# ha7ilm/csdr

Measured on AMD Instinct MI355X. Metric: complex MS/s in->out, WFM demod chain @2.4 MS/s x N streams, higher is better.
Workload: dtype f32

## Files before the change

### csdr_amd/csrc/wfm.hip

```cpp
#include "common.hpp"
#include "wfm_mfma.hpp"
#include "seeds.hpp"
#include <math.h>
#include <stdlib.h>
#include <vector>
#include <string>
#include <string.h>
using namespace csdr_amd;

namespace {

constexpr int HIST = WFM_HIST;
constexpr int TILE_A = 64;
constexpr int WARM = 48;

struct WfmParams {
    int D, L, F;
    int T;
    long long B;
    long long j_first;
    int n_audio;
};

__device__ __forceinline__ float u8_to_f(uint32_t v) { return fmaf((float)v, 0x1.010102p-7f, -1.0f); }
// ... 147 lines not shown
    long long B, next_j;
    int last_T, flip;
    bool ended;
    std::string kernel_name;
    bool profiling;
    std::vector<std::pair<hipEvent_t, hipEvent_t>> ev_pool;
    size_t ev_used;
    double prof_ms; long prof_launches;
    bool use_mfma;
    WfmMfmaDevice mfma;
    float2 *d_ctab; size_t ctab_cap;
    float2 c_prev;
    long long tab_first; bool tab_valid;
    bool ps; std::vector<float> rates, h_taps; csdr_amd::SeedTables *seeds; float *d_scales;
    float2 *d_dtab_old; int *d_list, *d_lead_n; float *d_lead_d; std::vector<int> retuned;
};

extern "C" {

static int wfm_upload_stream_tables(csdr_amd_wfm *w, int s, float rate)
{
    WfmMfmaTable t;
    wfm_mfma_build_table(w->D, w->L, w->F, rate, w->h_taps.data(), t);
    CSDR_HIP(hipMemcpy((uint8_t *)w->mfma.d_seq_frags + (size_t)s * t.seq_frags.size(), t.seq_frags.data(), t.seq_frags.size(), hipMemcpyHostToDevice));
    CSDR_HIP(hipMemcpy(w->mfma.d_seq_cum + (size_t)s * t.seq_cum.size(), t.seq_cum.data(), t.seq_cum.size() * sizeof(float), hipMemcpyHostToDevice));
    CSDR_HIP(hipMemcpy(w->mfma.d_dtab + (size_t)s * t.dtab.size(), t.dtab.data(), t.dtab.size() * sizeof(float2), hipMemcpyHostToDevice));
    CSDR_HIP(hipMemcpy(w->d_scales + s, &t.seq_scale, sizeof(float), hipMemcpyHostToDevice));
    return 0;
}

// ... 3 lines not shown
    const float shift_rate = rates ? rates[0] : 0.f;
    if (n_streams <= 0 || decimation <= 0 || taps_length <= 0 || frac_rate <= 1 || !rates) { fail_msg(-3, "wfm: bad parameters"); return nullptr; }
    if (decimation * 1 + taps_length + 8 > HIST) { fail_msg(-3, "wfm: D + taps (%d + %d) exceed the %d-sample history", decimation, taps_length, HIST); return nullptr; }
    if (max_block_samples < 1024) max_block_samples = 1024;
    csdr_amd_wfm *w = new csdr_amd_wfm();
    w->ctx = ctx; w->n_streams = n_streams; w->D = decimation; w->L = taps_length; w->F = frac_rate; w->audio_rate = audio_rate;
    w->shift_rate = shift_rate; w->tau = tau; w->max_block = max_block_samples;
    const float dt = (float)(1.0 / audio_rate); w->alpha = dt / (tau + dt);
    const size_t max_audio = max_block_samples / ((size_t)decimation * frac_rate) + 8;
    w->demod_pitch = (max_audio + 40 + 63) & ~(size_t)63;
    hipError_t e = hipSuccess;
    auto alloc = [&](void **p, size_t bytes) { if (e == hipSuccess) e = hipMalloc(p, bytes); };
    w->d_demod = nullptr; w->d_rot = nullptr; w->d_hist = nullptr; w->d_head[0] = w->d_head[1] = nullptr; w->hflip = 0;
    w->use_mfma = false; w->d_ctab = nullptr; w->ctab_cap = 0; w->mfma.d_seq_frags = nullptr; w->mfma.d_seq_cum = nullptr; w->mfma.d_dtab = nullptr;
    w->ps = per_stream; w->seeds = nullptr; w->d_scales = nullptr; w->d_dtab_old = nullptr; w->d_list = nullptr; w->d_lead_n = nullptr; w->d_lead_d = nullptr;
    {
        const char *force = getenv("CSDR_AMD_WFM_PATH");
        w->use_mfma = !(force && !strcmp(force, "valu")) && wfm_mfma_supported(decimation, taps_length, frac_rate);
    }
    if (per_stream && !w->use_mfma) { fail_msg(-3, "wfm_create_rates: a rate per stream needs the matrix-core chain kernel (decimation x audio decimation even, window <= 256 samples)"); delete w; return nullptr; }
    alloc((void **)&w->d_taps, sizeof(float) * taps_length);
    alloc((void **)&w->d_last[0], sizeof(float) * n_streams);
    alloc((void **)&w->d_last[1], sizeof(float) * n_streams);
    if (w->use_mfma) {
        alloc((void **)&w->d_head[0], wfm_mfma_head_bytes(n_streams));
        alloc((void **)&w->d_head[1], wfm_mfma_head_bytes(n_streams));
    } else {
        alloc((void **)&w->d_demod, sizeof(float) * w->demod_pitch * n_streams);
        alloc((void **)&w->d_rot, sizeof(cf32) * (HIST + max_block_samples + 64));
        alloc((void **)&w->d_hist, (size_t)2 * HIST * n_streams);
    }
    if (e != hipSuccess) { fail(e, "hipMalloc(wfm state)", __FILE__, __LINE__); csdr_amd_wfm_destroy(w); return nullptr; }
    (void)hipMemcpy(w->d_taps, host_taps, sizeof(float) * taps_length, hipMemcpyHostToDevice);
    w->kernel_name = "k_wfm_front";
    if (w->use_mfma && per_stream) {
        WfmMfmaTable t;
        wfm_mfma_build_table(decimation, taps_length, frac_rate, shift_rate, host_taps, t);
        w->mfma.tile_stride_bytes = t.tile_stride_bytes; w->mfma.win_off_bytes = t.win_off_bytes; w->mfma.seq_scale = t.seq_scale;
        w->rates.assign(rates, rates + n_streams); w->h_taps.assign(host_taps, host_taps + taps_length);
        hipError_t e2 = hipMalloc(&w->mfma.d_seq_frags, t.seq_frags.size() * (size_t)n_streams);
        if (e2 == hipSuccess) e2 = hipMalloc((void **)&w->mfma.d_seq_cum, t.seq_cum.size() * sizeof(float) * (size_t)n_streams);
// ... 51 lines not shown
    }
    const int rc = wfm_upload_stream_tables(w, stream, shift_rate); if (rc) return rc;
    w->rates[stream] = shift_rate;
    return seeds_set_rate(w->seeds, stream, shift_rate, false);
}

float csdr_amd_wfm_get_rate(const csdr_amd_wfm *w, int stream) { return w->ps ? ((stream >= 0 && stream < w->n_streams) ? w->rates[stream] : 0.f) : w->shift_rate; }

void csdr_amd_wfm_destroy(csdr_amd_wfm *w)
{
    if (!w) return;
    (void)hipStreamSynchronize(w->ctx->stream);
    if (w->seeds) seeds_destroy(w->seeds);
    (void)hipFree(w->d_scales); (void)hipFree(w->d_dtab_old); (void)hipFree(w->d_lead_n); (void)hipFree(w->d_lead_d);
    (void)hipFree(w->d_taps); (void)hipFree(w->d_demod); (void)hipFree(w->d_last[0]); (void)hipFree(w->d_last[1]);
    (void)hipFree(w->d_rot); (void)hipFree(w->d_hist); (void)hipFree(w->d_head[0]); (void)hipFree(w->d_head[1]);
    for (auto &pr : w->ev_pool) { (void)hipEventDestroy(pr.first); (void)hipEventDestroy(pr.second); }
    (void)hipFree(w->mfma.d_seq_frags); (void)hipFree(w->mfma.d_seq_cum); (void)hipFree(w->mfma.d_dtab); (void)hipFree(w->d_ctab);
    delete w;
}

int csdr_amd_wfm_reset(csdr_amd_wfm *w)
{
    hipStream_t st = w->ctx->stream;
    w->phase = 0.f;
    CSDR_HIP(hipMemsetAsync(w->d_last[0], 0, sizeof(float) * w->n_streams, st));
    CSDR_HIP(hipMemsetAsync(w->d_last[1], 0, sizeof(float) * w->n_streams, st));
    if (w->d_rot) CSDR_HIP(hipMemsetAsync(w->d_rot, 0, sizeof(cf32) * (HIST + w->max_block + 64), st));
    if (w->d_hist) CSDR_HIP(hipMemsetAsync(w->d_hist, 0x80, (size_t)2 * HIST * w->n_streams, st));
    for (int k = 0; k < 2; k++) if (w->d_head[k]) CSDR_HIP(hipMemsetAsync(w->d_head[k], 0x80, wfm_mfma_head_bytes(w->n_streams), st));
    w->hflip = 0;
// ... 113 lines not shown
                if (n_lead > n_audio) n_lead = n_audio;
            }
            if (n_lead > 0) {
                const int nr = (int)w->retuned.size(), S = w->n_streams;
                if (!w->d_lead_n) { CSDR_HIP(hipMalloc((void **)&w->d_lead_n, sizeof(int) * 2 * S)); w->d_list = w->d_lead_n + S; CSDR_HIP(hipMalloc((void **)&w->d_lead_d, sizeof(float) * (size_t)lead_max * S)); }
                int *hl = (int *)c->pinned_acquire(sizeof(int) * (size_t)(S + nr)); if (!hl) return -2;
                for (int s = 0; s < S; s++) hl[s] = 0;
                for (int k = 0; k < nr; k++) { hl[w->retuned[k]] = (int)n_lead; hl[S + k] = w->retuned[k]; }
                rc = c->pinned_upload(w->d_lead_n, sizeof(int) * (size_t)(S + nr)); if (rc) return rc;
                rc = wfm_mfma_lead(st, in, in_pitch, back.head_in, w->d_taps, sv.ctab, sv.pitch, w->mfma.d_dtab, w->d_dtab_old, w->d_list, nr, w->d_lead_d, lead_max,
                                   w->D, w->L, w->F, w->B, w->next_j, (int)n_lead);
                if (rc) return rc;
                psa.d_lead_d = w->d_lead_d; psa.d_lead_n = w->d_lead_n;
            }
        }
        rc = wfm_mfma_launch(st, e0, e1, in, in_pitch, w->mfma, ctab_call, w->n_streams, T, w->B, w->next_j, n_audio, back, w->ps ? &psa : nullptr);
        if (rc) return rc;
        if (n_audio > 0) w->retuned.clear();
        w->hflip ^= 1;
        if (n_audio > 0) w->flip ^= 1;
    } else {
        if ((size_t)n_audio + 40 > w->demod_pitch) return fail_msg(-3, "wfm: internal audio buffer too small");
        if (n_audio > 0) {
            WfmParams p; p.D = w->D; p.L = w->L; p.F = w->F; p.T = T; p.B = w->B; p.j_first = w->next_j; p.n_audio = n_audio;
            const int span = w->D * (w->F * (TILE_A - 1) + 1) + w->L + 16;
            const size_t lds = (size_t)((span + 7) / 8 * 8 + 2 * TILE_A) * sizeof(float2) + 64;
            if (lds > 64 * 1024) { const int arc = lds_attr_once((const void *)k_wfm_front, lds); if (arc) return arc; }
            if (e0) CSDR_HIP(hipEventRecord(e0, st));
            hipLaunchKernelGGL(k_wfm_front, dim3(w->n_streams, cdiv(n_audio, TILE_A)), dim3(256), lds, st,
                               in, in_pitch, w->d_hist, w->d_rot, w->d_taps, w->d_demod, w->demod_pitch, p);
            CSDR_LAUNCH_CHECK();
// ... 18 lines not shown
```

### csdr_amd/csrc/wfm_mfma.hip

```cpp
#include "common.hpp"
#include "wfm_mfma.hpp"
#include <hip/hip_ext.h>
#include <math.h>
#include <string.h>
#include <stdlib.h>
#include <complex>
#include <vector>
using namespace csdr_amd;

namespace csdr_amd {

bool wfm_mfma_supported(int D, int L, int F)
{
    if ((D * F) & 1) return false;
    const int win_off = (18 * D) & ~15;
    const int span_bytes = 2 * (D * (3 * F + 10) + L) - win_off;
    if (span_bytes > 64 * WFM_NK) return false;
    if (D + L + 3 * D * F + 8 > WFM_HIST) return false;
    return true;
}

void wfm_mfma_build_table(int D, int L, int F, float shift_rate, const float *taps, WfmMfmaTable &t)
{
    t.D = D; t.L = L; t.F = F;
// ... 97 lines not shown
            for (int l = 0; l < 3; l++) acc[l] = __builtin_amdgcn_mfma_i32_16x16x64_i8(A[ks * 3 + l], Bf[ks], acc[l], 0, 0, 0);
        }
    }
}

struct SeqParams {
    int n_streams; long long B2; long long tile_first; int n_tiles, tiles_per_seg;
    int stride, win_off; float scale;
    long long two_T;
    float alpha; const float *last_in; float *last_out; int16_t *s16; float *af; size_t out_pitch; long long j_first; int n_audio;
    const uint8_t *head_in; uint8_t *head_out;
    long long col_bytes; int col_chunks, col_audio, n_cols;
    size_t frag_stride, tab_pitch; int tab_len;
    const float *scales;
    const float *lead_d; const int *lead_n; int lead_stride;
};

#ifndef SEQ_RB_KIB
#define SEQ_RB_KIB 9
#endif
constexpr int SEQ_RB = 1024 * SEQ_RB_KIB;
#ifndef SEQ_RING_PAD
#define SEQ_RING_PAD 32
#endif
constexpr int SEQ_RP = SEQ_RB + SEQ_RING_PAD;
constexpr int SEQ_NGR = 4 * WFM_NK;
#ifndef SEQ_TPG_N
#define SEQ_TPG_N 6
#endif
#ifndef SEQ_NLD_N
// ... 4 lines not shown
constexpr int SEQ_NW = SEQ_TPG + SEQ_NLD;
constexpr int SEQ_NLW = SEQ_NLD;
constexpr int SEQ_LINE = 64;
constexpr int SEQ_OUTS = (SEQ_LINE - 1 + 3 * 4 * SEQ_TPG + 4 * SEQ_TPG - 1) / (4 * SEQ_TPG);
constexpr int SEQ_OUTR = SEQ_OUTS * 4 * SEQ_TPG;
constexpr int SEQ_OUTP = SEQ_OUTR + 4;
static_assert(16 % SEQ_NLW == 0 && (16 / SEQ_NLW) * 7 <= 63 && SEQ_TPG % 2 == 0, "rows per fetching wave (vmcnt counts to 63); the de-emphasis scan works on pairs");
constexpr int SEQ_HEAD = 1024;

#ifndef WFM_DIAG
#define WFM_DIAG 0
#endif
#ifdef WFM_PROF
__device__ unsigned long long g_wfm_prof[SEQ_NW][8];
__device__ unsigned long long g_wfm_life[SEQ_NW][4];
#define PROF_T(k) { const long long t_now = __builtin_readcyclecounter(); prof[k] += t_now - t_prev; t_prev = t_now; }
#else
#define PROF_T(k)
#endif

constexpr int RES_WARM = 48;
struct ResCtl {
    const uint32_t *desc;
    const uint32_t *ctrl;
    uint32_t *done;
    unsigned *cnt;
    unsigned long long *t_first;
    unsigned long long *next_item;
    unsigned *exiting;
    const uint8_t *in_ring; int16_t *out_ring; size_t in_slot_bytes, out_slot_elems;
    int n_slots, desc_lines, n_wsb, T, D, L, F;
    long long idle_ticks, life_ticks;
    const float *lead_d; int lead_stride;
    const float *lead_state;
    unsigned long long *stats;
    int fence_mode;
};
__device__ __forceinline__ uint32_t sys_load(const uint32_t *p) { return __hip_atomic_load(p, __ATOMIC_RELAXED, __HIP_MEMORY_SCOPE_SYSTEM); }
__device__ __forceinline__ uint32_t res_tag(long long k) { return (uint32_t)((unsigned long long)k % 0xfffffffeull) + 1u; }

template <bool PS, bool RES = false>
__global__ __launch_bounds__(64 * SEQ_NW) void k_wfm_mfma_seq(const uint8_t *__restrict__ in, size_t in_pitch, const v4i *__restrict__ frags, const float *__restrict__ cum,
                                                               const float2 *__restrict__ dtab, const float2 *__restrict__ ctab, SeqParams p_in, ResCtl rc)
{
    static_assert(!(PS && RES), "the resident form exists for the shared-rate kernel");
    constexpr int TPG = SEQ_TPG, SPW = 16 / SEQ_NLW, NTHR = 64 * SEQ_NW;
    extern __shared__ float4 lds_raw[];
    uint8_t *lds_in = reinterpret_cast<uint8_t *>(lds_raw);
    float *lds_out = reinterpret_cast<float *>(lds_in + 16 * SEQ_RP);
    float *lcum = lds_out + 16 * SEQ_OUTP;
    float2 *ctl = reinterpret_cast<float2 *>(lcum + (SEQ_NGR + 1) * 16);
    const int tid = threadIdx.x, wv = __builtin_amdgcn_readfirstlane(tid >> 6), lane = tid & 63, col = lane & 15, q = lane >> 4;
    const bool fetches = wv >= TPG;
#ifdef WFM_PROF
    const long long t_entry = __builtin_readcyclecounter();
    long long t_first = t_entry, t_last = t_entry;
#endif
    const int fw = wv - TPG;
    float scale = p_in.scale;
    if constexpr (PS) { const int sbp = blockIdx.x; frags += (size_t)sbp * p_in.frag_stride; cum += (size_t)sbp * ((SEQ_NGR + 1) * 16); dtab += (size_t)sbp * 3072; ctab += sbp; scale = p_in.scales[sbp]; }
    for (int i = tid; i < (SEQ_NGR + 1) * 16; i += NTHR) lcum[i] = cum[i];
    v4i A[WFM_NK * 3];
#pragma unroll
    for (int s = 0; s < WFM_NK * 3; s++) A[s] = frags[s * 64 + lane];

    float c_lo[4], c_hi[4];
    {
        const float4 a = *reinterpret_cast<const float4 *>(cum + 4 * q), b = *reinterpret_cast<const float4 *>(cum + (size_t)SEQ_NGR * 16 + 4 * q);
        c_lo[0] = a.x; c_lo[1] = a.y; c_lo[2] = a.z; c_lo[3] = a.w; c_hi[0] = b.x; c_hi[1] = b.y; c_hi[2] = b.z; c_hi[3] = b.w;
    }
    const float K = 0.340447550238101026565118445432744920253753662109375f;
    SeqParams p_res;
    if constexpr (RES) p_res = p_in;
    const SeqParams &p = RES ? p_res : p_in;
    unsigned long long item = 0;
    long long res_t_launch = 0;
    uint32_t *const rctl = reinterpret_cast<uint32_t *>(ctl);
    const float2 *const lseed = ctl + 1;
    long long st_wait = 0, st_body = 0, st_done = 0, st_items = 0, st_t = 0;
    if constexpr (RES) { item = rc.next_item[blockIdx.x]; res_t_launch = wall_clock64(); st_t = res_t_launch; }
    bool pend = false; unsigned pend_c = 0; int pend_slot = 0, pend_n = 0; long long pend_k = 0;
    uint32_t pre_v[4] = {0u, 0u, 0u, 0u}; bool pre_valid = false;
// ... 3 lines not shown
                pend = false;
                if (pend_c + 1 == (unsigned)rc.n_wsb) {
                    const unsigned long long tf = __hip_atomic_exchange(rc.t_first + pend_slot, ~0ull, __ATOMIC_RELAXED, __HIP_MEMORY_SCOPE_AGENT), td = (unsigned long long)wall_clock64();
                    __hip_atomic_store(rc.cnt + pend_slot, 0u, __ATOMIC_RELAXED, __HIP_MEMORY_SCOPE_AGENT);
                    uint32_t *dn = rc.done + (size_t)pend_slot * 16;
                    __hip_atomic_store(dn + 1, (uint32_t)pend_n, __ATOMIC_RELAXED, __HIP_MEMORY_SCOPE_SYSTEM);
                    __hip_atomic_store(dn + 2, (uint32_t)tf, __ATOMIC_RELAXED, __HIP_MEMORY_SCOPE_SYSTEM); __hip_atomic_store(dn + 3, (uint32_t)(tf >> 32), __ATOMIC_RELAXED, __HIP_MEMORY_SCOPE_SYSTEM);
                    __hip_atomic_store(dn + 4, (uint32_t)td, __ATOMIC_RELAXED, __HIP_MEMORY_SCOPE_SYSTEM); __hip_atomic_store(dn + 5, (uint32_t)(td >> 32), __ATOMIC_RELAXED, __HIP_MEMORY_SCOPE_SYSTEM);
                    asm volatile("s_waitcnt vmcnt(0)" ::: "memory");
                    __hip_atomic_store(dn, res_tag(pend_k), __ATOMIC_RELAXED, __HIP_MEMORY_SCOPE_SYSTEM);
                }
            }
        }
    };
    for (;;) {
    int res_slot = 0, res_lead = 0; long long res_k = 0; bool res_retuned = false;
    const uint8_t *pblock = nullptr;
    if constexpr (RES) {
        res_k = (long long)(item / (unsigned)rc.n_wsb);
        res_slot = (int)(res_k % rc.n_slots);
        if (wv == 0) {
            const uint32_t *dsc = rc.desc + (size_t)res_slot * rc.desc_lines * 16;
            const uint32_t tag = res_tag(res_k);
            const int nd = rc.desc_lines * 16;
            const long long t_wait = wall_clock64();
            uint32_t state = 0;
            for (int iter = 0;; iter++) {
                uint32_t v[4] = {0u, 0u, 0u, 0u};
                bool have = false;
                if (iter == 0 && pre_valid) {
// ... 46 lines not shown
        auto j_hi = [&](long long kk) -> long long {
            if (kk < 0) return -1;
            const long long avail_last = (kk + 1) * rc.T - 1;
            if (avail_last - (rc.L - 1) < 0) return -1;
            const long long k_max = (avail_last - (rc.L - 1)) / rc.D;
            return k_max >= 10 ? (k_max - 10) / rc.F : -1;
        };
        const long long jp = j_hi(res_k - 1), jn = j_hi(res_k);
        p_res.B2 = 2 * res_k * rc.T;
        p_res.j_first = jp + 1; p_res.n_audio = (int)(jn - jp);
        p_res.tile_first = p_res.j_first / 4; p_res.n_tiles = (int)((p_res.j_first + p_res.n_audio - 1) / 4 - p_res.tile_first + 1);
        p_res.tiles_per_seg = p_res.n_tiles;
        p_res.s16 = rc.out_ring + (size_t)res_slot * rc.out_slot_elems;
        if (tid == 0) (void)__hip_atomic_fetch_min(rc.t_first + res_slot, (unsigned long long)wall_clock64(), __ATOMIC_RELAXED, __HIP_MEMORY_SCOPE_AGENT);
    }
    const int sb = RES ? (int)(item % (unsigned)rc.n_wsb) : (int)blockIdx.x;
    const int seg_y = RES ? 0 : (int)blockIdx.y;
    const int col0 = PS ? 16 * seg_y : 0;
    if constexpr (RES) {
        in = rc.in_ring + (size_t)res_slot * rc.in_slot_bytes;
        pblock = rc.in_ring + (size_t)((res_slot + rc.n_slots - 1) % rc.n_slots) * rc.in_slot_bytes + (long long)sb * 16 * (long long)in_pitch;
    }
    const long long t0 = p.tile_first + (long long)seg_y * p.tiles_per_seg * (PS ? 16 : 1);
    long long t1 = t0 + p.tiles_per_seg; if (t1 > p.tile_first + p.n_tiles) t1 = p.tile_first + p.n_tiles;
    if (!RES && t0 >= t1) return;
    const int n_it = (int)(t1 - t0), n_grp = (n_it + TPG - 1) / TPG;
    const int n_lead = RES ? res_lead : ((PS && p.lead_n && seg_y == 0) ? p.lead_n[sb] : 0);
    const int n_warm = RES ? ((res_k > 0 && !res_retuned) ? 2 : 0) : ((PS || seg_y > 0) ? 2 : 0);
    const int last_stream = p.n_streams - 1;
    const int tstride = p.stride;
    const long long org = PS ? (long long)col0 * p.col_bytes : 0LL;
    long long wg = (t0 - (long long)n_warm * TPG) * tstride + p.win_off - p.B2 - org;
    const long long F0 = wg & ~1023LL;
    long long F_end = ((t1 - 1) * tstride + p.win_off - p.B2 - org + 64 * WFM_NK + 1023) & ~1023LL;
    { const long long row_end = ((p.two_T + 1023) & ~1023LL) - org; if (F_end > row_end) F_end = row_end; }
    long long F = F0;
    int fslot = (int)((F0 + 2 * SEQ_RB) % SEQ_RB), wslot = (int)((wg + 2 * SEQ_RB) % SEQ_RB);
    const uint32_t lds_in_addr = (uint32_t)(size_t)(__attribute__((address_space(3))) uint8_t *)lds_in;
    uint32_t voff[SPW], voff_h[SPW];
    long long row_lim[SPW];
// ... 169 lines not shown
            const int srow = ei / SPS, k = ei % SPS, kr = g * SPS + k;
            if (ei >= 16 * SPS) continue;
            if (PS ? (kr < col_lo(srow) || kr >= col_hi(srow)) : (kr < seg_lo || kr >= seg_hi || s0 + srow >= p.n_streams)) continue;
            const float e = lds_out[srow * SEQ_OUTP + (g % SEQ_OUTS) * SPS + k];
            const long long idx = idx0 + kr;
            const size_t at = PS ? (size_t)sb * p.out_pitch + (size_t)srow * p.col_audio + idx : (size_t)(s0 + srow) * p.out_pitch + idx;
            p.s16[at] = (int16_t)s16_of(e);
            if (p.af) p.af[at] = e;
        }
    };
#ifdef WFM_PROF
    long long prof[8] = {0, 0, 0, 0, 0, 0, 0, 0}, t_prev = __builtin_readcyclecounter();
#endif
    if (fetches) {
        typedef unsigned wfm_u4 __attribute__((ext_vector_type(4)));
        constexpr int NST = RES ? 8 : 44;
#define WFM_ST_ALL(X) X(0) X(1) X(2) X(3) X(4) X(5) X(6) X(7) X(8) X(9) X(10) X(11) X(12) X(13) X(14) X(15) X(16) X(17) X(18) X(19) X(20) X(21) X(22) X(23) \
                      X(24) X(25) X(26) X(27) X(28) X(29) X(30) X(31) X(32) X(33) X(34) X(35) X(36) X(37) X(38) X(39) X(40) X(41) X(42) X(43)
#define X(k) wfm_u4 st##k = {0u, 0u, 0u, 0u};
        WFM_ST_ALL(X)
#undef X
        int n_st = 0, st_n0 = 0;
        const int srow = 8 * fw + (lane >> 3), pc = lane & 7;
        const int lo_r = col_lo(srow), hi_r = col_hi(srow);
        const bool row_ok = PS ? hi_r > lo_r : s0 + srow < p.n_streams;
        const size_t row_at = PS ? (size_t)sb * p.out_pitch + (size_t)srow * p.col_audio : (size_t)(s0 + srow) * p.out_pitch;
        int16_t *const orow = p.s16 + row_at;
        auto flush = [&]() __attribute__((always_inline)) {
            if constexpr (PS) {
#define X(j) if (j < NST && j < n_st && row_ok) { const int a = st_n0 + SEQ_LINE * j + 8 * pc;                                                             \
                 if (a + 8 <= hi_r) *reinterpret_cast<uint4 *>(orow + (idx0 + a)) = make_uint4(st##j[0], st##j[1], st##j[2], st##j[3]);        \
// ... 196 lines not shown
            }
        }
        PROF_T(5)
#ifdef WFM_PROF
        prof[6] += 1;
#endif
        wg = wg_n; wslot += TPG * tstride; if (wslot >= SEQ_RB) wslot -= SEQ_RB;
    }
#ifdef WFM_PROF
    if (lane == 0) for (int k = 0; k < 8; k++) atomicAdd(&g_wfm_prof[wv][k], (unsigned long long)prof[k]);
    t_last = __builtin_readcyclecounter();
#endif
    __syncthreads();
    if (!emit_vec) emit_scalar(n_grp - 1);
    }
    if (PS && seg_y + 1 == (int)gridDim.y) {
        if (iir_lane && col0 + lane == p.n_cols - 1) p.last_out[sb] = yst;
        if (tid < 32 && p.two_T >= 512 && (p.two_T & 15) == 0) {
            const uint4 v = *reinterpret_cast<const uint4 *>(in + (size_t)sb * in_pitch + (p.two_T - 512) + 16 * tid);
            *reinterpret_cast<uint4 *>(p.head_out + (size_t)sb * SEQ_HEAD + 512 + 16 * tid) = v;
        }
    } else
    if (!PS && !RES && seg_y + 1 == (int)gridDim.y) {
        if (iir_lane && s0 + lane < p.n_streams) p.last_out[s0 + lane] = yst;
        if (tid < 16 * 32 && p.two_T >= 512 && (p.two_T & 15) == 0 && s0 + tid / 32 < p.n_streams) {
            const int srow = tid / 32, piece = tid % 32;
            const uint4 v = *reinterpret_cast<const uint4 *>(sblock + (size_t)srow * in_pitch + (p.two_T - 512) + 16 * piece);
            *reinterpret_cast<uint4 *>(p.head_out + (size_t)(s0 + srow) * SEQ_HEAD + 512 + 16 * piece) = v;
        }
    }
#ifdef WFM_PROF
    if (lane == 0) {
        asm volatile("s_waitcnt vmcnt(0)" ::: "memory");
        const long long t_exit = __builtin_readcyclecounter();
        atomicAdd(&g_wfm_life[wv][0], (unsigned long long)(t_first - t_entry)); atomicAdd(&g_wfm_life[wv][1], (unsigned long long)(t_last - t_first));
        atomicAdd(&g_wfm_life[wv][2], (unsigned long long)(t_exit - t_last)); atomicAdd(&g_wfm_life[wv][3], 1ULL);
    }
#endif
    if constexpr (!RES) break;
    else {
        if (tid == 0) { const long long t = wall_clock64(); st_body += t - st_t; st_t = t; }
        if (wv == 0) {
            const unsigned long long nx = item + gridDim.x;
            const long long nk = (long long)(nx / (unsigned)rc.n_wsb);
            const uint32_t *dsc = rc.desc + (size_t)(nk % rc.n_slots) * rc.desc_lines * 16;
            const int nd = rc.desc_lines * 16;
#pragma unroll
            for (int j = 0; j < 4; j++) { const int d = lane + 64 * j; pre_v[j] = d < nd ? sys_load(dsc + d) : 0u; }
            pre_valid = true;
        }
        if (rc.fence_mode == 2) __threadfence_system();
        if (wv != 0 || !emit_vec) asm volatile("s_waitcnt vmcnt(0)" ::: "memory");
        __syncthreads();
        if (tid == 0) {
// ... 81 lines not shown
                         const float2 *d_dtab_old, const int *d_list, int n_list, float *d_lead_d, int lead_stride, float *d_warm, float *d_state, float alpha,
                         int D, int L, int F, long long B, long long j_first, int n_lead)
{
    if (n_list <= 0) return 0;
    if (j_first < RES_WARM) return fail_msg(-3, "wfm ring: a retune needs %d audio samples in front of the block", RES_WARM);
    LeadParams lp; lp.D = D; lp.L = L; lp.F = F; lp.B = B; lp.j_first = j_first; lp.n_lead = n_lead; lp.tab_pitch = 1; lp.dtab_stride = 0;
    lp.ct_stride = 0; lp.head_pitch = in_pitch; lp.head_off = two_T - 512; lp.c_first = (B >> 10) - 4; lp.ja0 = -RES_WARM; lp.warm = d_warm; lp.lead_stride = lead_stride;
    hipLaunchKernelGGL(k_wfm_lead, dim3(n_lead + RES_WARM, n_list), dim3(128), 0, st, in, in_pitch, prev, d_taps, ctab, d_dtab, d_dtab_old, d_list, d_lead_d, lp);
    CSDR_LAUNCH_CHECK();
    hipLaunchKernelGGL(k_wfm_lead_state, dim3((n_list + 63) / 64), dim3(64), 0, st, d_warm, d_state, n_list, alpha);
    CSDR_LAUNCH_CHECK();
    return 0;
}

int wfm_mfma_launch(hipStream_t st, hipEvent_t ev_begin, hipEvent_t ev_end, const uint8_t *in, size_t in_pitch, const WfmMfmaDevice &dev, const float2 *ctab,
                    int n_streams, int T, long long B, long long j_first, int n_audio, const WfmBackArgs &back, const WfmPerStream *ps)
{
    if (in_pitch * 16 + 4096 >= ((size_t)1 << 32)) return fail_msg(-3, "wfm: in_pitch %zu too large for the matrix-core front end (32-bit row offsets)", in_pitch);
    if (n_audio <= 0) {
        hipLaunchKernelGGL(k_wfm_roll_head, dim3(n_streams), dim3(256), 0, st, in, in_pitch, 2LL * T, back.head_in, back.head_out);
        CSDR_LAUNCH_CHECK();
        return 0;
    }
    SeqParams sp;
    memset((void *)&sp, 0, sizeof sp);
    ResCtl no_res; memset((void *)&no_res, 0, sizeof no_res);
    sp.n_streams = n_streams; sp.B2 = 2 * B; sp.two_T = 2LL * T;
    sp.tile_first = j_first / 4; sp.n_tiles = (int)((j_first + n_audio - 1) / 4 - sp.tile_first + 1);
    sp.stride = dev.tile_stride_bytes; sp.win_off = dev.win_off_bytes; sp.scale = dev.seq_scale;
    const int n_cu = current_device_cu_count();
    const int n_wsb = (n_streams + 15) / 16;
    int n_seg = (n_cu + n_wsb - 1) / n_wsb; if (n_seg < 1) n_seg = 1;
    if (n_seg > sp.n_tiles / 24) n_seg = sp.n_tiles / 24;
    if (n_seg < 1) n_seg = 1;
    sp.tiles_per_seg = ((sp.n_tiles + n_seg - 1) / n_seg + SEQ_TPG - 1) / SEQ_TPG * SEQ_TPG;
    n_seg = (sp.n_tiles + sp.tiles_per_seg - 1) / sp.tiles_per_seg;
    sp.alpha = back.alpha; sp.last_in = back.last_in; sp.last_out = back.last_out; sp.s16 = back.s16; sp.af = back.af; sp.out_pitch = back.out_pitch;
    sp.j_first = j_first; sp.n_audio = n_audio; sp.head_in = back.head_in; sp.head_out = back.head_out;
    if (ps) {
        const long long ts = sp.stride / 2;
        long long per = ts; { long long a = per, b = 1024; while (b) { const long long t = a % b; a = b; b = t; } per = per / a * 1024; }
        int tpp = (int)(per / ts);
        while ((4 * tpp) % SEQ_LINE) tpp *= 2;
        const int n_per = (sp.n_tiles + tpp - 1) / tpp;
        int n_ss = (4 * n_cu + n_streams - 1) / n_streams; if (n_ss < 1) n_ss = 1;
        int np = (n_per + 16 * n_ss - 1) / (16 * n_ss); if (np < 1) np = 1;
        sp.tiles_per_seg = np * tpp;
        sp.n_cols = (sp.n_tiles + sp.tiles_per_seg - 1) / sp.tiles_per_seg;
        n_seg = (sp.n_cols + 15) / 16;
        sp.col_bytes = (long long)sp.tiles_per_seg * sp.stride; sp.col_chunks = (int)(sp.col_bytes / 2048); sp.col_audio = 4 * sp.tiles_per_seg;
        sp.frag_stride = (size_t)WFM_NK * 3 * 64; sp.tab_pitch = ps->tab_pitch; sp.tab_len = ps->tab_len; sp.scales = ps->d_scales;
        sp.lead_d = ps->d_lead_d; sp.lead_n = ps->d_lead_n; sp.lead_stride = ps->lead_stride;
        if (sp.col_bytes * 16 + 4096 >= (1LL << 32)) return fail_msg(-3, "wfm: block too large for the per-stream kernel's 32-bit row offsets");
        const size_t ldsp = (size_t)16 * SEQ_RP + 16 * SEQ_OUTP * sizeof(float) + (SEQ_NGR + 1) * 16 * sizeof(float) + 2 * 48 * sizeof(float2);
        { const int arc = lds_attr_once((const void *)k_wfm_mfma_seq<true>, ldsp); if (arc) return arc; }
        if (ev_begin && ev_end)
            hipExtLaunchKernelGGL(k_wfm_mfma_seq<true>, dim3(n_streams, n_seg), dim3(64 * SEQ_NW), ldsp, st, ev_begin, ev_end, 0, in, in_pitch, (const v4i *)dev.d_seq_frags, dev.d_seq_cum, dev.d_dtab, ctab, sp, no_res);
        else
            hipLaunchKernelGGL(k_wfm_mfma_seq<true>, dim3(n_streams, n_seg), dim3(64 * SEQ_NW), ldsp, st, in, in_pitch, (const v4i *)dev.d_seq_frags, dev.d_seq_cum, dev.d_dtab, ctab, sp, no_res);
        CSDR_LAUNCH_CHECK();
        if (T < 256 || (T & 7)) {
            hipLaunchKernelGGL(k_wfm_roll_head, dim3(n_streams), dim3(256), 0, st, in, in_pitch, 2LL * T, back.head_in, back.head_out);
            CSDR_LAUNCH_CHECK();
        }
        return 0;
    }
    const size_t lds = (size_t)16 * SEQ_RP + 16 * SEQ_OUTP * sizeof(float) + (SEQ_NGR + 1) * 16 * sizeof(float);
    { const int arc = lds_attr_once((const void *)k_wfm_mfma_seq<false>, lds); if (arc) return arc; }
    if (ev_begin && ev_end)
        hipExtLaunchKernelGGL(k_wfm_mfma_seq<false>, dim3(n_wsb, n_seg), dim3(64 * SEQ_NW), lds, st, ev_begin, ev_end, 0, in, in_pitch, (const v4i *)dev.d_seq_frags, dev.d_seq_cum, dev.d_dtab, ctab, sp, no_res);
    else
        hipLaunchKernelGGL(k_wfm_mfma_seq<false>, dim3(n_wsb, n_seg), dim3(64 * SEQ_NW), lds, st, in, in_pitch, (const v4i *)dev.d_seq_frags, dev.d_seq_cum, dev.d_dtab, ctab, sp, no_res);
    CSDR_LAUNCH_CHECK();
    if (T < 256 || (T & 7)) {
        hipLaunchKernelGGL(k_wfm_roll_head, dim3(n_streams), dim3(256), 0, st, in, in_pitch, 2LL * T, back.head_in, back.head_out);
        CSDR_LAUNCH_CHECK();
    }
    return 0;
}

int wfm_mfma_launch_resident(hipStream_t st, hipEvent_t ev_end, const WfmMfmaDevice &dev, int n_streams, size_t in_pitch, float alpha, size_t out_pitch, const WfmResident &rv, int grid)
{
    if (in_pitch * 16 + 4096 >= ((size_t)1 << 32)) return fail_msg(-3, "wfm ring: in_pitch %zu too large (32-bit row offsets)", in_pitch);
    SeqParams sp; memset((void *)&sp, 0, sizeof sp);
    sp.n_streams = n_streams; sp.two_T = 2LL * rv.T; sp.stride = dev.tile_stride_bytes; sp.win_off = dev.win_off_bytes; sp.scale = dev.seq_scale;
    sp.alpha = alpha; sp.out_pitch = out_pitch;
    ResCtl rc; memset((void *)&rc, 0, sizeof rc);
    rc.desc = rv.desc; rc.ctrl = rv.ctrl; rc.done = rv.done; rc.cnt = rv.cnt; rc.t_first = rv.t_first; rc.next_item = rv.next_item; rc.exiting = rv.exiting;
// ... 14 lines not shown
}

#ifdef WFM_PROF
extern "C" int csdr_amd_debug_wfm_prof(unsigned long long *out, int reset)
{
    if (hipMemcpyFromSymbol(out, HIP_SYMBOL(g_wfm_prof), sizeof(unsigned long long) * SEQ_NW * 8) != hipSuccess) return -1;
    if (reset) { static unsigned long long z[SEQ_NW * 8]; if (hipMemcpyToSymbol(HIP_SYMBOL(g_wfm_prof), z, sizeof(z)) != hipSuccess) return -1; }
    return 0;
}
extern "C" int csdr_amd_debug_wfm_life(unsigned long long *out, int reset)
{
    if (hipMemcpyFromSymbol(out, HIP_SYMBOL(g_wfm_life), sizeof(unsigned long long) * SEQ_NW * 4) != hipSuccess) return -1;
    if (reset) { static unsigned long long z[SEQ_NW * 4]; if (hipMemcpyToSymbol(HIP_SYMBOL(g_wfm_life), z, sizeof(z)) != hipSuccess) return -1; }
    return 0;
}
#endif

extern "C" int csdr_amd_debug_wfm_seq_tile(int D, int L, int F, float shift_rate, const float *taps, long long n0, const uint8_t *window,
                                           const float *ctab2, float *out16)
{
    if (!wfm_mfma_supported(D, L, F) || (n0 & 7)) return -1;
    static WfmMfmaTable t; static int cD = 0, cL = 0, cF = 0; static float crate = 0; static std::vector<float> ctaps;
    if (cD != D || cL != L || cF != F || crate != shift_rate || ctaps != std::vector<float>(taps, taps + L)) {
        wfm_mfma_build_table(D, L, F, shift_rate, taps, t); cD = D; cL = L; cF = F; crate = shift_rate; ctaps.assign(taps, taps + L);
    }
    const int off = (int)(n0 & 1023);
    const bool two = off + 32 * WFM_NK > 1024;
    const int bo = 2 * (1024 - off), kb = two ? (bo >> 6) : WFM_NK, hq = (bo >> 4) & 3, gb = bo >> 4;
    const float2 D0 = t.dtab[off + 2048], C0 = make_float2(ctab2[0], ctab2[1]);
    const float2 P0 = make_float2(C0.x * D0.x - C0.y * D0.y, C0.x * D0.y + C0.y * D0.x);
// ... 33 lines not shown
```

### csdr_amd/csrc/wfm_mfma.hpp

```cpp
#pragma once
#include "common.hpp"
#include <vector>

namespace csdr_amd {

constexpr int WFM_HIST = 256;
constexpr int WFM_NK = 8;

struct WfmMfmaTable {
    int D, L, F, tile_stride_bytes, win_off_bytes;
    std::vector<int8_t> seq_frags;
    std::vector<float> seq_cum;
    std::vector<float2> dtab;
    float seq_scale;
};

struct WfmMfmaDevice {
    int tile_stride_bytes, win_off_bytes;
    void *d_seq_frags; float *d_seq_cum; float2 *d_dtab; float seq_scale;
};

struct WfmBackArgs {
    float alpha; const float *last_in; float *last_out; int16_t *s16; float *af; size_t out_pitch; const uint8_t *head_in; uint8_t *head_out;
};
// ... 8 lines not shown
    int n_slots, desc_lines, T, D, L, F;
    long long idle_ticks, life_ticks;
    const float *lead_d, *lead_state; int lead_stride;
    unsigned long long *stats; int fence_mode;
};
constexpr int WFM_RES_WARM = 48;
int wfm_mfma_launch_resident(hipStream_t st, hipEvent_t ev_end, const WfmMfmaDevice &dev, int n_streams, size_t in_pitch, float alpha, size_t out_pitch, const WfmResident &rv, int grid);
int wfm_resident_max_grid();
int wfm_mfma_lead_shared(hipStream_t st, const uint8_t *in, size_t in_pitch, const uint8_t *prev, size_t two_T, const float *d_taps, const float2 *ctab, const float2 *d_dtab,
                         const float2 *d_dtab_old, const int *d_list, int n_list, float *d_lead_d, int lead_stride, float *d_warm, float *d_state, float alpha,
                         int D, int L, int F, long long B, long long j_first, int n_lead);

bool wfm_mfma_supported(int D, int L, int F);
void wfm_mfma_build_table(int D, int L, int F, float shift_rate, const float *taps, WfmMfmaTable &t);
size_t wfm_mfma_head_bytes(int n_streams);
int wfm_mfma_launch(hipStream_t st, hipEvent_t ev_begin, hipEvent_t ev_end, const uint8_t *in, size_t in_pitch, const WfmMfmaDevice &dev, const float2 *ctab,
                    int n_streams, int T, long long B, long long j_first, int n_audio, const WfmBackArgs &back, const WfmPerStream *ps = nullptr);
int wfm_mfma_lead(hipStream_t st, const uint8_t *in, size_t in_pitch, const uint8_t *head, const float *d_taps, const float2 *ctab, size_t tab_pitch, const float2 *d_dtab,
                  const float2 *d_dtab_old, const int *d_list, int n_list, float *d_lead_d, int lead_stride, int D, int L, int F, long long B, long long j_first, int n_lead);

}
```

Before: 2.919 million.

## Add persistent work-walk grid for shared-rate WFM matrix-core kernel via atomic tickets

Adds a WALK variant of the shared-rate MFMA chain kernel. It launches one block per CU, and each block pulls (stream-block, segment) items from a global atomic ticket counter instead of using a 2D grid. Table fragments are reloaded per item, and the store-staging depth for fetch waves drops from 44 to 32. The aim is to remove tail and launch imbalance when there are more items than CUs. In exchange it adds an atomic and a barrier per item, plus repeated table loads. It is on by default and can be disabled with CSDR_AMD_WFM_WALK=0.

```diff
diff --git a/csdr_amd/csrc/wfm.hip b/csdr_amd/csrc/wfm.hip
--- a/csdr_amd/csrc/wfm.hip
+++ b/csdr_amd/csrc/wfm.hip
@@ -185,6 +185,7 @@
     long long tab_first; bool tab_valid;
     bool ps; std::vector<float> rates, h_taps; csdr_amd::SeedTables *seeds; float *d_scales;
     float2 *d_dtab_old; int *d_list, *d_lead_n; float *d_lead_d; std::vector<int> retuned;
+    WfmWalk walk;
 };
 
 extern "C" {
@@ -218,9 +219,12 @@
     w->d_demod = nullptr; w->d_rot = nullptr; w->d_hist = nullptr; w->d_head[0] = w->d_head[1] = nullptr; w->hflip = 0;
     w->use_mfma = false; w->d_ctab = nullptr; w->ctab_cap = 0; w->mfma.d_seq_frags = nullptr; w->mfma.d_seq_cum = nullptr; w->mfma.d_dtab = nullptr;
     w->ps = per_stream; w->seeds = nullptr; w->d_scales = nullptr; w->d_dtab_old = nullptr; w->d_list = nullptr; w->d_lead_n = nullptr; w->d_lead_d = nullptr;
+    w->walk.d_tickets = nullptr; w->walk.base = 0;
     {
         const char *force = getenv("CSDR_AMD_WFM_PATH");
         w->use_mfma = !(force && !strcmp(force, "valu")) && wfm_mfma_supported(decimation, taps_length, frac_rate);
+        const char *wk = getenv("CSDR_AMD_WFM_WALK");
+        w->walk.on = !(wk && !strcmp(wk, "0"));
     }
     if (per_stream && !w->use_mfma) { fail_msg(-3, "wfm_create_rates: a rate per stream needs the matrix-core chain kernel (decimation x audio decimation even, window <= 256 samples)"); delete w; return nullptr; }
     alloc((void **)&w->d_taps, sizeof(float) * taps_length);
@@ -229,6 +233,8 @@
     if (w->use_mfma) {
         alloc((void **)&w->d_head[0], wfm_mfma_head_bytes(n_streams));
         alloc((void **)&w->d_head[1], wfm_mfma_head_bytes(n_streams));
+        alloc((void **)&w->walk.d_tickets, sizeof(unsigned long long));
+        if (e == hipSuccess) e = hipMemset(w->walk.d_tickets, 0, sizeof(unsigned long long));
     } else {
         alloc((void **)&w->d_demod, sizeof(float) * w->demod_pitch * n_streams);
         alloc((void **)&w->d_rot, sizeof(cf32) * (HIST + max_block_samples + 64));
@@ -310,7 +316,7 @@
     if (w->seeds) seeds_destroy(w->seeds);
     (void)hipFree(w->d_scales); (void)hipFree(w->d_dtab_old); (void)hipFree(w->d_lead_n); (void)hipFree(w->d_lead_d);
     (void)hipFree(w->d_taps); (void)hipFree(w->d_demod); (void)hipFree(w->d_last[0]); (void)hipFree(w->d_last[1]);
-    (void)hipFree(w->d_rot); (void)hipFree(w->d_hist); (void)hipFree(w->d_head[0]); (void)hipFree(w->d_head[1]);
+    (void)hipFree(w->d_rot); (void)hipFree(w->d_hist); (void)hipFree(w->d_head[0]); (void)hipFree(w->d_head[1]); (void)hipFree(w->walk.d_tickets);
     for (auto &pr : w->ev_pool) { (void)hipEventDestroy(pr.first); (void)hipEventDestroy(pr.second); }
     (void)hipFree(w->mfma.d_seq_frags); (void)hipFree(w->mfma.d_seq_cum); (void)hipFree(w->mfma.d_dtab); (void)hipFree(w->d_ctab);
     delete w;
@@ -454,7 +460,7 @@
                 psa.d_lead_d = w->d_lead_d; psa.d_lead_n = w->d_lead_n;
             }
         }
-        rc = wfm_mfma_launch(st, e0, e1, in, in_pitch, w->mfma, ctab_call, w->n_streams, T, w->B, w->next_j, n_audio, back, w->ps ? &psa : nullptr);
+        rc = wfm_mfma_launch(st, e0, e1, in, in_pitch, w->mfma, ctab_call, w->n_streams, T, w->B, w->next_j, n_audio, back, w->ps ? &psa : nullptr, &w->walk);
         if (rc) return rc;
         if (n_audio > 0) w->retuned.clear();
         w->hflip ^= 1;
diff --git a/csdr_amd/csrc/wfm_mfma.hip b/csdr_amd/csrc/wfm_mfma.hip
--- a/csdr_amd/csrc/wfm_mfma.hip
+++ b/csdr_amd/csrc/wfm_mfma.hip
@@ -135,6 +135,7 @@
     size_t frag_stride, tab_pitch; int tab_len;
     const float *scales;
     const float *lead_d; const int *lead_n; int lead_stride;
+    unsigned long long *tickets; unsigned long long ticket_base; int n_items, n_x, n_seg;
 };
 
 #ifndef SEQ_RB_KIB
@@ -169,6 +170,7 @@
 #ifdef WFM_PROF
 __device__ unsigned long long g_wfm_prof[SEQ_NW][8];
 __device__ unsigned long long g_wfm_life[SEQ_NW][4];
+__device__ unsigned long long g_wfm_life_walk[SEQ_NW][4];
 #define PROF_T(k) { const long long t_now = __builtin_readcyclecounter(); prof[k] += t_now - t_prev; t_prev = t_now; }
 #else
 #define PROF_T(k)
@@ -194,33 +196,54 @@
 __device__ __forceinline__ uint32_t sys_load(const uint32_t *p) { return __hip_atomic_load(p, __ATOMIC_RELAXED, __HIP_MEMORY_SCOPE_SYSTEM); }
 __device__ __forceinline__ uint32_t res_tag(long long k) { return (uint32_t)((unsigned long long)k % 0xfffffffeull) + 1u; }
 
-template <bool PS, bool RES = false>
+template <bool PS, bool RES = false, bool WALK = false>
 __global__ __launch_bounds__(64 * SEQ_NW) void k_wfm_mfma_seq(const uint8_t *__restrict__ in, size_t in_pitch, const v4i *__restrict__ frags, const float *__restrict__ cum,
                                                                const float2 *__restrict__ dtab, const float2 *__restrict__ ctab, SeqParams p_in, ResCtl rc)
 {
     static_assert(!(PS && RES), "the resident form exists for the shared-rate kernel");
+    static_assert(!(RES && WALK), "the resident form has its own walk");
+    static_assert(!(PS && WALK), "a rate per stream reloads every table per item and holds four items per CU: nothing for a walk to save (DESIGN 4e)");
     constexpr int TPG = SEQ_TPG, SPW = 16 / SEQ_NLW, NTHR = 64 * SEQ_NW;
     extern __shared__ float4 lds_raw[];
     uint8_t *lds_in = reinterpret_cast<uint8_t *>(lds_raw);
     float *lds_out = reinterpret_cast<float *>(lds_in + 16 * SEQ_RP);
     float *lcum = lds_out + 16 * SEQ_OUTP;
     float2 *ctl = reinterpret_cast<float2 *>(lcum + (SEQ_NGR + 1) * 16);
+    int *const wslot_item = reinterpret_cast<int *>(ctl);
     const int tid = threadIdx.x, wv = __builtin_amdgcn_readfirstlane(tid >> 6), lane = tid & 63, col = lane & 15, q = lane >> 4;
     const bool fetches = wv >= TPG;
 #ifdef WFM_PROF
-    const long long t_entry = __builtin_readcyclecounter();
+    long long t_entry = __builtin_readcyclecounter();
     long long t_first = t_entry, t_last = t_entry;
+    bool prof_later = false;
 #endif
     const int fw = wv - TPG;
     float scale = p_in.scale;
+    auto draw = [&]() -> int {
+        if (tid == 0) {
+            const unsigned long long t = __hip_atomic_fetch_add(p_in.tickets, 1ull, __ATOMIC_RELAXED, __HIP_MEMORY_SCOPE_AGENT) - p_in.ticket_base;
+            *wslot_item = t < (unsigned long long)p_in.n_items ? (int)t : -1;
+        }
+        __syncthreads();
+        return __builtin_amdgcn_readfirstlane(*wslot_item);
+    };
+    int w_item = 0;
+    if constexpr (WALK) { w_item = draw(); if (w_item < 0) return; }
     if constexpr (PS) { const int sbp = blockIdx.x; frags += (size_t)sbp * p_in.frag_stride; cum += (size_t)sbp * ((SEQ_NGR + 1) * 16); dtab += (size_t)sbp * 3072; ctab += sbp; scale = p_in.scales[sbp]; }
-    for (int i = tid; i < (SEQ_NGR + 1) * 16; i += NTHR) lcum[i] = cum[i];
     v4i A[WFM_NK * 3];
-#pragma unroll
-    for (int s = 0; s < WFM_NK * 3; s++) A[s] = frags[s * 64 + lane];
-
     float c_lo[4], c_hi[4];
-    {
+    auto load_tables = [&]() __attribute__((always_inline)) {
+        if constexpr (WALK) { asm volatile("" : "+s"(frags), "+s"(cum)); }
+        for (int i = tid; i < (SEQ_NGR + 1) * 16; i += NTHR) lcum[i] = cum[i];
+#pragma unroll
+        for (int s = 0; s < WFM_NK * 3; s++) A[s] = frags[s * 64 + lane];
+        const float4 a = *reinterpret_cast<const float4 *>(cum + 4 * q), b = *reinterpret_cast<const float4 *>(cum + (size_t)SEQ_NGR * 16 + 4 * q);
+        c_lo[0] = a.x; c_lo[1] = a.y; c_lo[2] = a.z; c_lo[3] = a.w; c_hi[0] = b.x; c_hi[1] = b.y; c_hi[2] = b.z; c_hi[3] = b.w;
+    };
+    if constexpr (!WALK) {
+        for (int i = tid; i < (SEQ_NGR + 1) * 16; i += NTHR) lcum[i] = cum[i];
+#pragma unroll
+        for (int s = 0; s < WFM_NK * 3; s++) A[s] = frags[s * 64 + lane];
         const float4 a = *reinterpret_cast<const float4 *>(cum + 4 * q), b = *reinterpret_cast<const float4 *>(cum + (size_t)SEQ_NGR * 16 + 4 * q);
         c_lo[0] = a.x; c_lo[1] = a.y; c_lo[2] = a.z; c_lo[3] = a.w; c_hi[0] = b.x; c_hi[1] = b.y; c_hi[2] = b.z; c_hi[3] = b.w;
     }
@@ -254,6 +277,7 @@
         }
     };
     for (;;) {
+    if constexpr (WALK) load_tables();
     int res_slot = 0, res_lead = 0; long long res_k = 0; bool res_retuned = false;
     const uint8_t *pblock = nullptr;
     if constexpr (RES) {
@@ -330,8 +354,8 @@
         p_res.s16 = rc.out_ring + (size_t)res_slot * rc.out_slot_elems;
         if (tid == 0) (void)__hip_atomic_fetch_min(rc.t_first + res_slot, (unsigned long long)wall_clock64(), __ATOMIC_RELAXED, __HIP_MEMORY_SCOPE_AGENT);
     }
-    const int sb = RES ? (int)(item % (unsigned)rc.n_wsb) : (int)blockIdx.x;
-    const int seg_y = RES ? 0 : (int)blockIdx.y;
+    const int sb = RES ? (int)(item % (unsigned)rc.n_wsb) : WALK ? w_item % p.n_x : (int)blockIdx.x;
+    const int seg_y = RES ? 0 : WALK ? w_item / p.n_x : (int)blockIdx.y;
     const int col0 = PS ? 16 * seg_y : 0;
     if constexpr (RES) {
         in = rc.in_ring + (size_t)res_slot * rc.in_slot_bytes;
@@ -339,7 +363,10 @@
     }
     const long long t0 = p.tile_first + (long long)seg_y * p.tiles_per_seg * (PS ? 16 : 1);
     long long t1 = t0 + p.tiles_per_seg; if (t1 > p.tile_first + p.n_tiles) t1 = p.tile_first + p.n_tiles;
-    if (!RES && t0 >= t1) return;
+    if (!RES && t0 >= t1) {
+        if constexpr (!WALK) return;
+        else { w_item = draw(); if (w_item < 0) return; continue; }
+    }
     const int n_it = (int)(t1 - t0), n_grp = (n_it + TPG - 1) / TPG;
     const int n_lead = RES ? res_lead : ((PS && p.lead_n && seg_y == 0) ? p.lead_n[sb] : 0);
     const int n_warm = RES ? ((res_k > 0 && !res_retuned) ? 2 : 0) : ((PS || seg_y > 0) ? 2 : 0);
@@ -539,7 +566,7 @@
 #endif
     if (fetches) {
         typedef unsigned wfm_u4 __attribute__((ext_vector_type(4)));
-        constexpr int NST = RES ? 8 : 44;
+        constexpr int NST = RES ? 8 : WALK ? 32 : 44;
 #define WFM_ST_ALL(X) X(0) X(1) X(2) X(3) X(4) X(5) X(6) X(7) X(8) X(9) X(10) X(11) X(12) X(13) X(14) X(15) X(16) X(17) X(18) X(19) X(20) X(21) X(22) X(23) \
                       X(24) X(25) X(26) X(27) X(28) X(29) X(30) X(31) X(32) X(33) X(34) X(35) X(36) X(37) X(38) X(39) X(40) X(41) X(42) X(43)
 #define X(k) wfm_u4 st##k = {0u, 0u, 0u, 0u};
@@ -766,14 +793,15 @@
     __syncthreads();
     if (!emit_vec) emit_scalar(n_grp - 1);
     }
-    if (PS && seg_y + 1 == (int)gridDim.y) {
+    const int n_seg = WALK ? p.n_seg : (int)gridDim.y;
+    if (PS && seg_y + 1 == n_seg) {
         if (iir_lane && col0 + lane == p.n_cols - 1) p.last_out[sb] = yst;
         if (tid < 32 && p.two_T >= 512 && (p.two_T & 15) == 0) {
             const uint4 v = *reinterpret_cast<const uint4 *>(in + (size_t)sb * in_pitch + (p.two_T - 512) + 16 * tid);
             *reinterpret_cast<uint4 *>(p.head_out + (size_t)sb * SEQ_HEAD + 512 + 16 * tid) = v;
         }
     } else
-    if (!PS && !RES && seg_y + 1 == (int)gridDim.y) {
+    if (!PS && !RES && seg_y + 1 == n_seg) {
         if (iir_lane && s0 + lane < p.n_streams) p.last_out[s0 + lane] = yst;
         if (tid < 16 * 32 && p.two_T >= 512 && (p.two_T & 15) == 0 && s0 + tid / 32 < p.n_streams) {
             const int srow = tid / 32, piece = tid % 32;
@@ -785,11 +813,18 @@
     if (lane == 0) {
         asm volatile("s_waitcnt vmcnt(0)" ::: "memory");
         const long long t_exit = __builtin_readcyclecounter();
-        atomicAdd(&g_wfm_life[wv][0], (unsigned long long)(t_first - t_entry)); atomicAdd(&g_wfm_life[wv][1], (unsigned long long)(t_last - t_first));
-        atomicAdd(&g_wfm_life[wv][2], (unsigned long long)(t_exit - t_last)); atomicAdd(&g_wfm_life[wv][3], 1ULL);
-    }
-#endif
-    if constexpr (!RES) break;
+        unsigned long long *lf = prof_later ? g_wfm_life_walk[wv] : g_wfm_life[wv];
+        atomicAdd(&lf[0], (unsigned long long)(t_first - t_entry)); atomicAdd(&lf[1], (unsigned long long)(t_last - t_first));
+        atomicAdd(&lf[2], (unsigned long long)(t_exit - t_last)); atomicAdd(&lf[3], 1ULL);
+    }
+#endif
+    if constexpr (WALK) {
+#ifdef WFM_PROF
+        t_entry = __builtin_readcyclecounter(); prof_later = true;
+#endif
+        w_item = draw();
+        if (w_item < 0) return;
+    } else if constexpr (!RES) break;
     else {
         if (tid == 0) { const long long t = wall_clock64(); st_body += t - st_t; st_t = t; }
         if (wv == 0) {
@@ -901,7 +936,7 @@
 }
 
 int wfm_mfma_launch(hipStream_t st, hipEvent_t ev_begin, hipEvent_t ev_end, const uint8_t *in, size_t in_pitch, const WfmMfmaDevice &dev, const float2 *ctab,
-                    int n_streams, int T, long long B, long long j_first, int n_audio, const WfmBackArgs &back, const WfmPerStream *ps)
+                    int n_streams, int T, long long B, long long j_first, int n_audio, const WfmBackArgs &back, const WfmPerStream *ps, WfmWalk *walk)
 {
     if (in_pitch * 16 + 4096 >= ((size_t)1 << 32)) return fail_msg(-3, "wfm: in_pitch %zu too large for the matrix-core front end (32-bit row offsets)", in_pitch);
     if (n_audio <= 0) {
@@ -924,6 +959,21 @@
     n_seg = (sp.n_tiles + sp.tiles_per_seg - 1) / sp.tiles_per_seg;
     sp.alpha = back.alpha; sp.last_in = back.last_in; sp.last_out = back.last_out; sp.s16 = back.s16; sp.af = back.af; sp.out_pitch = back.out_pitch;
     sp.j_first = j_first; sp.n_audio = n_audio; sp.head_in = back.head_in; sp.head_out = back.head_out;
+    auto walks = [&](int n_x, int n_seg_) {
+        if (!walk || !walk->on || !walk->d_tickets || (long long)n_x * n_seg_ <= n_cu) return false;
+        sp.tickets = walk->d_tickets; sp.ticket_base = walk->base; sp.n_items = n_x * n_seg_; sp.n_x = n_x; sp.n_seg = n_seg_;
+        return true;
+    };
+    auto launch = [&](const void *attr_key, auto kern, dim3 grid, size_t lds_bytes) -> int {
+        { const int arc = lds_attr_once(attr_key, lds_bytes); if (arc) return arc; }
+        if (ev_begin && ev_end)
+            hipExtLaunchKernelGGL(kern, grid, dim3(64 * SEQ_NW), lds_bytes, st, ev_begin, ev_end, 0, in, in_pitch, (const v4i *)dev.d_seq_frags, dev.d_seq_cum, dev.d_dtab, ctab, sp, no_res);
+        else
+            hipLaunchKernelGGL(kern, grid, dim3(64 * SEQ_NW), lds_bytes, st, in, in_pitch, (const v4i *)dev.d_seq_frags, dev.d_seq_cum, dev.d_dtab, ctab, sp, no_res);
+        CSDR_LAUNCH_CHECK();
+        if (sp.tickets) walk->base += (unsigned long long)sp.n_items + grid.x;
+        return 0;
+    };
     if (ps) {
         const long long ts = sp.stride / 2;
         long long per = ts; { long long a = per, b = 1024; while (b) { const long long t = a % b; a = b; b = t; } per = per / a * 1024; }
@@ -940,12 +990,7 @@
         sp.lead_d = ps->d_lead_d; sp.lead_n = ps->d_lead_n; sp.lead_stride = ps->lead_stride;
         if (sp.col_bytes * 16 + 4096 >= (1LL << 32)) return fail_msg(-3, "wfm: block too large for the per-stream kernel's 32-bit row offsets");
         const size_t ldsp = (size_t)16 * SEQ_RP + 16 * SEQ_OUTP * sizeof(float) + (SEQ_NGR + 1) * 16 * sizeof(float) + 2 * 48 * sizeof(float2);
-        { const int arc = lds_attr_once((const void *)k_wfm_mfma_seq<true>, ldsp); if (arc) return arc; }
-        if (ev_begin && ev_end)
-            hipExtLaunchKernelGGL(k_wfm_mfma_seq<true>, dim3(n_streams, n_seg), dim3(64 * SEQ_NW), ldsp, st, ev_begin, ev_end, 0, in, in_pitch, (const v4i *)dev.d_seq_frags, dev.d_seq_cum, dev.d_dtab, ctab, sp, no_res);
-        else
-            hipLaunchKernelGGL(k_wfm_mfma_seq<true>, dim3(n_streams, n_seg), dim3(64 * SEQ_NW), ldsp, st, in, in_pitch, (const v4i *)dev.d_seq_frags, dev.d_seq_cum, dev.d_dtab, ctab, sp, no_res);
-        CSDR_LAUNCH_CHECK();
+        { const int rc = launch((const void *)k_wfm_mfma_seq<true>, k_wfm_mfma_seq<true>, dim3(n_streams, n_seg), ldsp); if (rc) return rc; }
         if (T < 256 || (T & 7)) {
             hipLaunchKernelGGL(k_wfm_roll_head, dim3(n_streams), dim3(256), 0, st, in, in_pitch, 2LL * T, back.head_in, back.head_out);
             CSDR_LAUNCH_CHECK();
@@ -953,12 +998,13 @@
         return 0;
     }
     const size_t lds = (size_t)16 * SEQ_RP + 16 * SEQ_OUTP * sizeof(float) + (SEQ_NGR + 1) * 16 * sizeof(float);
-    { const int arc = lds_attr_once((const void *)k_wfm_mfma_seq<false>, lds); if (arc) return arc; }
-    if (ev_begin && ev_end)
-        hipExtLaunchKernelGGL(k_wfm_mfma_seq<false>, dim3(n_wsb, n_seg), dim3(64 * SEQ_NW), lds, st, ev_begin, ev_end, 0, in, in_pitch, (const v4i *)dev.d_seq_frags, dev.d_seq_cum, dev.d_dtab, ctab, sp, no_res);
-    else
-        hipLaunchKernelGGL(k_wfm_mfma_seq<false>, dim3(n_wsb, n_seg), dim3(64 * SEQ_NW), lds, st, in, in_pitch, (const v4i *)dev.d_seq_frags, dev.d_seq_cum, dev.d_dtab, ctab, sp, no_res);
-    CSDR_LAUNCH_CHECK();
+    if (walks(n_wsb, n_seg)) {
+        const int rc = launch((const void *)k_wfm_mfma_seq<false, false, true>, k_wfm_mfma_seq<false, false, true>, dim3(n_cu), lds + 16);
+        if (rc) return rc;
+    } else {
+        const int rc = launch((const void *)k_wfm_mfma_seq<false>, k_wfm_mfma_seq<false>, dim3(n_wsb, n_seg), lds);
+        if (rc) return rc;
+    }
     if (T < 256 || (T & 7)) {
         hipLaunchKernelGGL(k_wfm_roll_head, dim3(n_streams), dim3(256), 0, st, in, in_pitch, 2LL * T, back.head_in, back.head_out);
         CSDR_LAUNCH_CHECK();
@@ -1003,6 +1049,12 @@
     if (reset) { static unsigned long long z[SEQ_NW * 4]; if (hipMemcpyToSymbol(HIP_SYMBOL(g_wfm_life), z, sizeof(z)) != hipSuccess) return -1; }
     return 0;
 }
+extern "C" int csdr_amd_debug_wfm_life_walk(unsigned long long *out, int reset)
+{
+    if (hipMemcpyFromSymbol(out, HIP_SYMBOL(g_wfm_life_walk), sizeof(unsigned long long) * SEQ_NW * 4) != hipSuccess) return -1;
+    if (reset) { static unsigned long long z[SEQ_NW * 4]; if (hipMemcpyToSymbol(HIP_SYMBOL(g_wfm_life_walk), z, sizeof(z)) != hipSuccess) return -1; }
+    return 0;
+}
 #endif
 
 extern "C" int csdr_amd_debug_wfm_seq_tile(int D, int L, int F, float shift_rate, const float *taps, long long n0, const uint8_t *window,
diff --git a/csdr_amd/csrc/wfm_mfma.hpp b/csdr_amd/csrc/wfm_mfma.hpp
--- a/csdr_amd/csrc/wfm_mfma.hpp
+++ b/csdr_amd/csrc/wfm_mfma.hpp
@@ -46,8 +46,9 @@
 bool wfm_mfma_supported(int D, int L, int F);
 void wfm_mfma_build_table(int D, int L, int F, float shift_rate, const float *taps, WfmMfmaTable &t);
 size_t wfm_mfma_head_bytes(int n_streams);
+struct WfmWalk { unsigned long long *d_tickets; unsigned long long base; bool on; };
 int wfm_mfma_launch(hipStream_t st, hipEvent_t ev_begin, hipEvent_t ev_end, const uint8_t *in, size_t in_pitch, const WfmMfmaDevice &dev, const float2 *ctab,
-                    int n_streams, int T, long long B, long long j_first, int n_audio, const WfmBackArgs &back, const WfmPerStream *ps = nullptr);
+                    int n_streams, int T, long long B, long long j_first, int n_audio, const WfmBackArgs &back, const WfmPerStream *ps = nullptr, WfmWalk *walk = nullptr);
 int wfm_mfma_lead(hipStream_t st, const uint8_t *in, size_t in_pitch, const uint8_t *head, const float *d_taps, const float2 *ctab, size_t tab_pitch, const float2 *d_dtab,
                   const float2 *d_dtab_old, const int *d_list, int n_list, float *d_lead_d, int lead_stride, int D, int L, int F, long long B, long long j_first, int n_lead);
 
```

Result: no change. 2.919 million (median of 6 runs) (+0.0%).
